# kch3782/torcwa

Measured on AMD Instinct MI355X. Metric: RCWA layer-solves/sec (complex64 I/O) at Fourier order [15,15], higher is better.
Workload: dtype c128 results (mixed-precision eigensolver: fp32 eigendecomposition refined to fp64 by two Newton steps -- fp64 residual and update GEMMs, the correction solved with ONE fp32 LU of the fp32 start; everything else fp64 MFMA); complex64 I/O; 1 GPU; configs[1]: single patterned layer, order=[15,15] (n=1922), 300x300 grid, 128-lambda sweep, glass input half-space; points_total=128, points_per_gpu=128, layer_solves_per_point=1, chunk=128, streams=1, precision=high

## Files before the change

include/trx.h:

```cpp
#ifndef TRX_H_
#define TRX_H_
#include <stddef.h>

#ifdef __cplusplus
extern "C" {
#endif

enum { TRX_C64 = 0, TRX_C128 = 1 };
enum { TRX_OP_N = 0, TRX_OP_T = 1, TRX_OP_C = 2 };
enum {
    TRX_OK = 0,
    TRX_ERR_DTYPE = -1,
    TRX_ERR_ARG = -2,
    TRX_ERR_WORKSPACE = -3,
    TRX_ERR_LAUNCH = -4,
    TRX_ERR_UNSUPPORTED = -5
};

int trx_version(void);
const char* trx_strerror(int code);

size_t trx_convmat_ws_bytes(int dtype, int batch, int nx, int ny, int ox, int oy);
int trx_convmat(int dtype, int grid_is_complex, const void* grid, int batch, int nx, int ny, int ox, int oy,
                void* out, void* ws, size_t ws_bytes, void* stream);
// ... 29 lines not shown
size_t trx_eig_ws_bytes(int dtype, int n, int batch);
int trx_eig(int dtype, void* A, void* w, void* V, int n, int batch, int* info, void* ws, size_t ws_bytes,
            void* stream);
int trx_eig_last_fallback(void);
size_t trx_eig_ws_bytes_opts(int dtype, int n, int batch, unsigned opts);
int trx_eig_opts(int dtype, void* A, void* w, void* V, int n, int batch, int* info, void* ws, size_t ws_bytes, void* stream, unsigned opts);

int trx_tuning(const char* key, int value);

size_t trx_eig_backward_ws_bytes(int dtype, int n, int batch);
int trx_eig_backward(int dtype, const void* w, const void* V, const void* gw, const void* gV, double broadening, int n, int batch,
                     void* gA, int* piv, int* info, void* ws, size_t ws_bytes, void* stream);

int trx_build_pq(int dtype, const void* E, const void* Einv, const void* Mu, const void* Muinv, const void* kx,
                 const void* ky, int N, int batch, void* P, void* Q, void* stream);

size_t trx_layer_smatrix_ws_bytes(int dtype, int N, int batch);
size_t trx_layer_smatrix_ws_bytes_lean(int dtype, int N, int batch);
size_t trx_hmodes_ws_bytes(int dtype, int N, int batch);
int trx_hmodes(int dtype, const void* E, const void* mu, const void* kx, const void* ky, const void* W, const void* kz, int N, int batch,
               void* V, int* piv, int* info, void* ws, size_t ws_bytes, void* stream);
int trx_layer_smatrix(int dtype, const void* P, const void* Q, const void* W, const void* kzfac, const void* vfinv,
                      const void* phase, int use_q, int N, int batch, void* S11, void* S21, void* V, void* Cplus,
                      void* Cminus, int* piv, int* info, void* ws, size_t ws_bytes, void* stream);

size_t trx_redheffer_ws_bytes(int dtype, int n, int batch);
int trx_redheffer(int dtype, const void* const* Sm, const void* const* Sn, void* const* Sout, void* XY, int n, int batch,
                  int* piv, int* info, void* ws, size_t ws_bytes, void* stream);

size_t trx_redheffer_halfspace_ws_bytes(int dtype, int N, int batch, int side, int want_xy);
int trx_redheffer_halfspace(int dtype, int side, const void* bd, const void* const* S, void* const* Sout, void* XY, int N, int batch,
                            int* piv, int* info, void* ws, size_t ws_bytes, void* stream);

size_t trx_build_a_ws_bytes(int dtype, int N, int batch);
int trx_build_a(int dtype, const void* E, const void* Einv, const void* mu, const void* kx, const void* ky, int N, int batch, void* A,
                void* ws, size_t ws_bytes, void* stream);

int trx_build_pq_aniso(int dtype, const void* Ex, const void* Ey, const void* Einv, const void* Mx, const void* My, const void* Minv,
                       const void* kx, const void* ky, int N, int batch, void* P, void* Q, void* stream);
size_t trx_build_a_aniso_ws_bytes(int dtype, int N, int batch);
int trx_build_a_aniso(int dtype, const void* Ex, const void* Ey, const void* Einv, const void* mu, const void* kx, const void* ky, int N, int batch,
                      void* A, void* ws, size_t ws_bytes, void* stream);

int trx_build_pq_tensor(int dtype, const void* Exx, const void* Exy, const void* Eyy, const void* Einv, const void* Mu, const void* Muinv,
                        const void* kx, const void* ky, int N, int batch, void* P, void* Q, void* stream);
size_t trx_build_a_tensor_ws_bytes(int dtype, int N, int batch);
int trx_build_a_tensor(int dtype, const void* Exx, const void* Exy, const void* Eyy, const void* Einv, const void* mu, const void* kx, const void* ky,
                       int N, int batch, void* A, void* ws, size_t ws_bytes, void* stream);

int trx_matvec(int dtype, const void* A, const void* X, long strideX, void* Y, int m, int k, int c, int batch, void* stream);
size_t trx_layer_flux_ws_bytes(int dtype, int N, int nz, int batch);
int trx_layer_flux(int dtype, const void* W, const void* V, const void* cplus, const void* cminus, const void* kz, const double* omega,
                   const double* d, const double* z, int z_is_fraction, int N, int nz, int batch, double* flux, void* ws, size_t ws_bytes,
                   void* stream);

int trx_prof_enable(int on);
int trx_prof_reset(void);
int trx_prof_get(int tag, double* out);
const char* trx_prof_tag_name(int tag);

#ifdef __cplusplus
}
#endif
#endif
```

torcwa_amd/_lib.py:

```python
import ctypes
import os
from ctypes import c_char_p, c_double, c_int, c_long, c_size_t, c_void_p

_HERE = os.path.dirname(os.path.abspath(__file__))
LIB_PATH = os.path.join(_HERE, "libtrx.so")

C64, C128 = 0, 1
OP_N, OP_T, OP_C = 0, 1, 2

_SIGS = {
    "trx_version": (c_int, []),
    "trx_strerror": (c_char_p, [c_int]),
    "trx_convmat_ws_bytes": (c_size_t, [c_int, c_int, c_int, c_int, c_int, c_int]),
    "trx_convmat": (c_int, [c_int, c_int, c_void_p, c_int, c_int, c_int, c_int, c_int, c_void_p, c_void_p, c_size_t, c_void_p]),
    "trx_convmat_orders_ws_bytes": (c_size_t, [c_int, c_int, c_int, c_int, c_int, c_int, c_int]),
    "trx_convmat_orders": (c_int, [c_int, c_int, c_void_p, c_int, c_int, c_int, c_void_p, c_int, c_int, c_int, c_void_p, c_void_p, c_size_t,
                                   c_void_p]),
    "trx_convmat_li_ws_bytes": (c_size_t, [c_int, c_int, c_int, c_int, c_int, c_int]),
    "trx_convmat_li": (c_int, [c_int, c_int, c_void_p, c_int, c_int, c_int, c_int, c_int, c_void_p, c_void_p, c_void_p, c_void_p, c_void_p,
                               c_void_p, c_size_t, c_void_p]),
    "trx_build_pq_aniso": (c_int, [c_int, c_void_p, c_void_p, c_void_p, c_void_p, c_void_p, c_void_p, c_void_p, c_void_p, c_int, c_int, c_void_p,
                                   c_void_p, c_void_p]),
    "trx_build_a_aniso_ws_bytes": (c_size_t, [c_int, c_int, c_int]),
    "trx_build_a_aniso": (c_int, [c_int, c_void_p, c_void_p, c_void_p, c_void_p, c_void_p, c_void_p, c_int, c_int, c_void_p, c_void_p, c_size_t,
# ... 1 lines not shown
    "trx_normal_field_ws_bytes": (c_size_t, [c_int, c_int, c_int, c_int]),
    "trx_normal_field": (c_int, [c_int, c_int, c_void_p, c_int, c_int, c_int, c_double, c_double, c_double, c_void_p, c_void_p, c_size_t, c_void_p]),
    "trx_convmat_nv_ws_bytes": (c_size_t, [c_int, c_int, c_int, c_int, c_int, c_int]),
    "trx_convmat_nv": (c_int, [c_int, c_int, c_void_p, c_int, c_int, c_int, c_int, c_int, c_double, c_double, c_double, c_void_p, c_void_p, c_void_p,
                               c_void_p, c_void_p, c_void_p, c_size_t, c_void_p]),
    "trx_normal_field_lattice": (c_int, [c_int, c_int, c_void_p, c_int, c_int, c_int, c_double, c_void_p, c_void_p, c_void_p, c_size_t, c_void_p]),
    "trx_convmat_nv_orders_ws_bytes": (c_size_t, [c_int, c_int, c_int, c_int, c_int, c_int, c_int]),
    "trx_convmat_nv_orders": (c_int, [c_int, c_int, c_void_p, c_int, c_int, c_int, c_void_p, c_int, c_int, c_int, c_double, c_void_p, c_void_p,
                                      c_void_p, c_void_p, c_void_p, c_void_p, c_void_p, c_size_t, c_void_p]),
    "trx_build_pq_tensor": (c_int, [c_int, c_void_p, c_void_p, c_void_p, c_void_p, c_void_p, c_void_p, c_void_p, c_void_p, c_int, c_int, c_void_p,
                                    c_void_p, c_void_p]),
    "trx_build_a_tensor_ws_bytes": (c_size_t, [c_int, c_int, c_int]),
    "trx_build_a_tensor": (c_int, [c_int, c_void_p, c_void_p, c_void_p, c_void_p, c_void_p, c_void_p, c_void_p, c_int, c_int, c_void_p, c_void_p,
                                   c_size_t, c_void_p]),
    "trx_gemm": (c_int, [c_int, c_int, c_int, c_int, c_int, c_int, c_void_p, c_void_p, c_int, c_long, c_void_p, c_int, c_long,
                         c_void_p, c_void_p, c_int, c_long, c_int, c_void_p]),
    "trx_lu_solve": (c_int, [c_int, c_void_p, c_int, c_void_p, c_int, c_int, c_void_p, c_void_p, c_void_p]),
    "trx_inverse_ws_bytes": (c_size_t, [c_int, c_int, c_int]),
    "trx_inverse": (c_int, [c_int, c_void_p, c_int, c_int, c_void_p, c_void_p, c_void_p, c_size_t, c_void_p]),
    "trx_eig_ws_bytes": (c_size_t, [c_int, c_int, c_int]),
    "trx_build_pq": (c_int, [c_int, c_void_p, c_void_p, c_void_p, c_void_p, c_void_p, c_void_p, c_int, c_int, c_void_p, c_void_p, c_void_p]),
    "trx_layer_smatrix_ws_bytes": (c_size_t, [c_int, c_int, c_int]),
    "trx_layer_smatrix_ws_bytes_lean": (c_size_t, [c_int, c_int, c_int]),
    "trx_layer_smatrix": (c_int, [c_int, c_void_p, c_void_p, c_void_p, c_void_p, c_void_p, c_void_p, c_int, c_int, c_int, c_void_p, c_void_p,
                                  c_void_p, c_void_p, c_void_p, c_void_p, c_void_p, c_void_p, c_size_t, c_void_p]),
    "trx_eig_backward_ws_bytes": (c_size_t, [c_int, c_int, c_int]),
    "trx_eig_backward": (c_int, [c_int, c_void_p, c_void_p, c_void_p, c_void_p, c_double, c_int, c_int, c_void_p, c_void_p, c_void_p, c_void_p, c_size_t, c_void_p]),
    "trx_hmodes_ws_bytes": (c_size_t, [c_int, c_int, c_int]),
    "trx_hmodes": (c_int, [c_int, c_void_p, c_void_p, c_void_p, c_void_p, c_void_p, c_void_p, c_int, c_int, c_void_p, c_void_p, c_void_p, c_void_p, c_size_t, c_void_p]),
    "trx_redheffer_ws_bytes": (c_size_t, [c_int, c_int, c_int]),
    "trx_redheffer": (c_int, [c_int, c_void_p, c_void_p, c_void_p, c_void_p, c_int, c_int, c_void_p, c_void_p, c_void_p, c_size_t, c_void_p]),
    "trx_redheffer_halfspace_ws_bytes": (c_size_t, [c_int, c_int, c_int, c_int, c_int]),
    "trx_redheffer_halfspace": (c_int, [c_int, c_int, c_void_p, c_void_p, c_void_p, c_void_p, c_int, c_int, c_void_p, c_void_p, c_void_p, c_size_t, c_void_p]),
    "trx_build_a_ws_bytes": (c_size_t, [c_int, c_int, c_int]),
    "trx_build_a": (c_int, [c_int, c_void_p, c_void_p, c_void_p, c_void_p, c_void_p, c_int, c_int, c_void_p, c_void_p, c_size_t, c_void_p]),
    "trx_matvec": (c_int, [c_int, c_void_p, c_void_p, c_long, c_void_p, c_int, c_int, c_int, c_int, c_void_p]),
    "trx_layer_flux_ws_bytes": (c_size_t, [c_int, c_int, c_int, c_int]),
    "trx_layer_flux": (c_int, [c_int, c_void_p, c_void_p, c_void_p, c_void_p, c_void_p, c_void_p, c_void_p, c_void_p, c_int, c_int, c_int, c_int,
                               c_void_p, c_void_p, c_size_t, c_void_p]),
    "trx_tuning": (c_int, [c_char_p, c_int]),
    "trx_prof_enable": (c_int, [c_int]),
    "trx_prof_reset": (c_int, []),
    "trx_prof_get": (c_int, [c_int, c_void_p]),
    "trx_prof_tag_name": (c_char_p, [c_int]),
    "trx_eig": (c_int, [c_int, c_void_p, c_void_p, c_void_p, c_int, c_int, c_void_p, c_void_p, c_size_t, c_void_p]),
    "trx_eig_last_fallback": (c_int, []),
    "trx_eig_ws_bytes_opts": (c_size_t, [c_int, c_int, c_int, ctypes.c_uint]),
    "trx_eig_opts": (c_int, [c_int, c_void_p, c_void_p, c_void_p, c_int, c_int, c_void_p, c_void_p, c_size_t, c_void_p, ctypes.c_uint]),
}


class TrxError(RuntimeError):
    pass


class TrxLib:

    def __init__(self, path):
        if not os.path.exists(path):
            raise TrxError(
                f"{path} not found: the HIP extension is not built. Run `python torcwa_amd/csrc/build.py` "
                "(hipcc --offload-arch=gfx950). torcwa_amd has no CPU fallback.")
        self.path = path
        self.dll = ctypes.CDLL(path)
        for name, (res, args) in _SIGS.items():
            fn = getattr(self.dll, name)
# ... 22 lines not shown
```

torcwa_amd/batched.py:

```python
import warnings

import numpy as np
import torch

from .engine import Engine, default_engine
from . import autograd_ops as ag
from . import lattice as _lat
from .flux import FluxMixin
from .torch_eig import Eig

PI_REF = 3.141592652589793

_DIRS = {"f": "forward", "forward": "forward", "b": "backward", "backward": "backward"}
_PORTS = {"t": "transmission", "transmission": "transmission", "r": "reflection", "reflection": "reflection"}
_SBLOCK = {("forward", "transmission"): 0, ("forward", "reflection"): 1, ("backward", "reflection"): 2, ("backward", "transmission"): 3}
_KZ_SIDES = {0: ("out", "in"), 1: ("in", "in"), 2: ("out", "out"), 3: ("in", "out")}
FOURIER_RULES = ("laurent", "li", "normal")
NV_SIGMA_DEFAULT = 6.0


def check_fourier_rule(rule):
    if rule not in FOURIER_RULES:
        raise ValueError(f"fourier_rule must be one of {FOURIER_RULES}, got {rule!r}")

# ... 547 lines not shown
                Cn[1].append(eng.gemm(C[1][m], Y2.contiguous()))
        return Sn, Cn

    @staticmethod
    def _is_bd(S):
        return isinstance(S[0], BlockDiag2)

    @staticmethod
    def _RS_bd_bd(Sm, Sn):
        one, zero = torch.ones_like(Sm[0].d[0]), torch.zeros_like(Sm[0].d[0])
        I = BlockDiag2(one, zero, zero, one)
        t1 = (I - Sm[2] @ Sn[1]).inv()
        t2 = (I - Sn[1] @ Sm[2]).inv()
        return [Sn[0] @ t1 @ Sm[0], Sm[1] + Sm[3] @ t2 @ Sn[1] @ Sm[0], Sn[2] + Sn[0] @ t1 @ Sm[2] @ Sn[3], Sm[3] @ t2 @ Sn[3]]

    def _star(self, Sm, Sn, Cm, Cn):
        bm, bn = self._is_bd(Sm), self._is_bd(Sn)
        if bm and bn:
            return self._RS_bd_bd(Sm, Sn), [[], []]
        if bm:
            return self._RS_halfspace(0, Sm, Sn, Cn)
        if bn:
            return self._RS_halfspace(1, Sn, Sm, Cm)
        return self._RS_prod(Sm, Sn, Cm, Cn)

    def _layer_S(self, i):
        return [self.layer_S11[i], self.layer_S21[i], self.layer_S21[i], self.layer_S11[i]]

    def _layer_C(self, i):
        if not self.keep_coupling or self.Cplus[i] is None:
            return [[], []]
        return [[torch.cat((self.Cplus[i], self.Cminus[i]), dim=1)], [torch.cat((self.Cminus[i], self.Cplus[i]), dim=1)]]

    def solve_global_smatrix(self):
        n, B = self.n, self.B
        self._zero_layer_S = False
        first = 1
        if self._n_folded > 0:
            S, C, first = self._running, [[], []], self._n_folded
        elif self.layer_N > 0:
            S = self._layer_S(0)
            C = self._layer_C(0)
        else:
            I = torch.eye(n, dtype=self._cdtype, device=self._device).expand(B, -1, -1).contiguous()
            Z = torch.zeros((B, n, n), dtype=self._cdtype, device=self._device)
            S = [I, Z, Z.clone(), I.clone()]
            C = [[], []]
            self._zero_layer_S = not (self.has_in or self.has_out)
        for i in range(first, self.layer_N):
            S, C = self._star(S, self._layer_S(i), C, self._layer_C(i))
        if self.has_in:
            S, C = self._star(self._Sin, S, [[], []], C)
        if self.has_out:
            S, C = self._star(S, self._Sout, C, [[], []])
        if self._is_bd(S):
            S = [blk.dense().to(self._cdtype) for blk in S]
        self.S = S
        self.C = C

    def _matching_indices(self, orders):
        if self._general:
            idx = []
            for p, q in orders.reshape(-1, 2).tolist():
                if (p, q) not in self._index:
                    raise ValueError(f"harmonic ({p}, {q}) is not in this solver's order set")
                idx.append(self._index[(p, q)])
            return torch.as_tensor(idx, dtype=torch.int64, device=orders.device)
        ox, oy = self.order
        orders[orders[:, 0] < -ox, 0] = -ox
        orders[orders[:, 0] > ox, 0] = ox
        orders[orders[:, 1] < -oy, 1] = -oy
        orders[orders[:, 1] > oy, 1] = oy
        return len(self.order_y) * (orders[:, 0] + ox) + orders[:, 1] + oy

    def _kz_real(self, side, evan, abs_when_evanescent=False):
        em = self.eps_in * self.mu_in if side == "in" else self.eps_out * self.mu_out
        kzc = torch.sqrt(em[:, None] - self.Kx_norm_dn ** 2 - self.Ky_norm_dn ** 2)
        ev = torch.abs(torch.real(kzc) / torch.imag(kzc)) < evan
        repl = torch.abs(torch.real(kzc)) if abs_when_evanescent else torch.zeros_like(torch.real(kzc))
        kz = torch.where(ev, repl, torch.real(kzc))
        return torch.cat((kz, kz), dim=1)

    def S_parameters(self, orders, *, direction="forward", port="transmission", polarization="xx", ref_order=[0, 0],
                     power_norm=True, evanscent=1e-3):
        dev = self._device
        orders = torch.as_tensor(orders, dtype=torch.int64, device=dev).reshape([-1, 2])
        if direction in _DIRS:
            direction = _DIRS[direction]
        else:
            warnings.warn("Invalid propagation direction. Set as forward.", UserWarning)
            direction = "forward"
        if port in _PORTS:
            port = _PORTS[port]
        else:
            warnings.warn("Invalid port. Set as tramsmission.", UserWarning)
            port = "transmission"
        if polarization not in ("xx", "yx", "xy", "yy", "pp", "sp", "ps", "ss"):
            warnings.warn("Invalid polarization. Set as xx.", UserWarning)
            polarization = "xx"
        ref_order = torch.as_tensor(ref_order, dtype=torch.int64, device=dev).reshape([1, 2])
        oi = self._matching_indices(orders)
        ri = self._matching_indices(ref_order)
        N = self.order_N
        k = _SBLOCK[(direction, port)]
        Sk = self.S[k]
        num_side, den_side = _KZ_SIDES[k]

        if polarization in ("xx", "yx", "xy", "yy"):
            if polarization[0] == "y":
                oi = oi + N
            if polarization[1] == "y":
                ri = ri + N
            val = Sk[:, oi, ri[0]]
            if power_norm:
                kzn, kzd = self._kz_real(num_side, evanscent), self._kz_real(den_side, evanscent)
                kxr = torch.cat((torch.real(self.Kx_norm_dn),) * 2, dim=1)
                kyr = torch.cat((torch.real(self.Ky_norm_dn),) * 2, dim=1)
                pn = kxr if polarization[0] == "x" else kyr
                pd = kxr if polarization[1] == "x" else kyr
                norm = torch.sqrt((1 + (pn[:, oi] / kzn[:, oi]) ** 2) / (1 + (pd[:, ri] / kzd[:, ri]) ** 2))
                norm = norm * torch.sqrt(kzn[:, oi] / kzd[:, ri])
                val = val * norm
            val = torch.where(torch.isinf(val), torch.zeros_like(val), val)
            val = torch.where(torch.isnan(val), torch.zeros_like(val), val)
            return val.to(self._dtype)

        osign, rsign = {0: (1, 1), 1: (-1, 1), 2: (1, -1), 3: (-1, -1)}[k]
        em_in, em_out = self.eps_in * self.mu_in, self.eps_out * self.mu_out
        ok2 = {0: em_out, 1: em_in, 2: em_out, 3: em_in}[k]
        rk2 = {0: em_in, 1: em_in, 2: em_out, 3: em_out}[k]

        def angles(idx, k2, sign):
            kx_, ky_ = self.Kx_norm_dn[:, idx], self.Ky_norm_dn[:, idx]
            kt = torch.sqrt(kx_ ** 2 + ky_ ** 2)
            kzc = torch.sqrt(k2[:, None] - kx_ ** 2 - ky_ ** 2)
            kzs = sign * torch.abs(torch.real(kzc))
            ev = torch.abs(torch.real(kzc) / torch.imag(kzc)) < evanscent
            return torch.atan2(torch.real(kt), kzs), torch.atan2(torch.real(ky_), torch.real(kx_)), ev

        o_inc, o_azi, o_ev = angles(oi, ok2, osign)
        r_inc, r_azi, r_ev = angles(ri, rk2, rsign)
        r0 = int(ri[0])
        xx, xy = Sk[:, oi, r0], Sk[:, oi, r0 + N]
        yx, yy = Sk[:, oi + N, r0], Sk[:, oi + N, r0 + N]
        zero = torch.zeros_like(xx)
        xx, xy, yx, yy = (torch.where(o_ev, zero, t) for t in (xx, xy, yx, yy))
        co, so, ci = torch.cos(o_azi), torch.sin(o_azi), torch.cos(o_inc)
        cr, sr, cri = torch.cos(r_azi), torch.sin(r_azi), torch.cos(r_inc)
        if polarization == "pp":
            val = co / ci * cri * cr * xx + so / ci * cri * cr * yx + co / ci * cri * sr * xy + so / ci * cri * sr * yy
        elif polarization == "ps":
            val = co / ci * (-1) * sr * xx + so / ci * (-1) * sr * yx + co / ci * cr * xy + so / ci * cr * yy
        elif polarization == "sp":
            val = -so * cri * cr * xx + co * cri * cr * yx + -so * cri * sr * xy + co * cri * sr * yy
        else:
            val = -so * (-1) * sr * xx + co * (-1) * sr * yx + -so * cr * xy + co * cr * yy
        val = torch.where(torch.isinf(val), torch.zeros_like(val), val)
        val = torch.where(torch.isnan(val), torch.zeros_like(val), val)
        if power_norm:
            kz_in = self._kz_real("in", evanscent)
            kz_out = self._kz_real("out", evanscent, abs_when_evanescent=True)
            kzn = kz_out if num_side == "out" else kz_in
            kzd = kz_out if den_side == "out" else kz_in
            val = val * torch.sqrt(kzn[:, oi] / kzd[:, ri])
        val = torch.where(r_ev, torch.zeros_like(val), val)
        return val.to(self._dtype)

    def diffraction_angle(self, orders, *, layer="output", unit="radian"):
        orders = torch.as_tensor(orders, dtype=torch.int64, device=self._device).reshape([-1, 2])
        if layer in ("i", "in", "input"):
            layer = "input"
        elif layer in ("o", "out", "output"):
            layer = "output"
        else:
            warnings.warn("Invalid layer. Set as output layer.", UserWarning)
            layer = "output"
        if unit in ("r", "rad", "radian"):
# ... 18 lines not shown
```

torcwa_amd/csrc/api.hip:

```cpp
#include "common.hpp"

using namespace trx;

extern "C" int trx_version(void) { return 500; }

extern "C" const char* trx_strerror(int code) {
    switch (code) {
        case TRX_OK: return "ok";
        case TRX_ERR_DTYPE: return "unsupported dtype (expected TRX_C64 or TRX_C128)";
        case TRX_ERR_ARG: return "invalid argument";
        case TRX_ERR_WORKSPACE: return "workspace too small";
        case TRX_ERR_LAUNCH: return "kernel launch failed";
        case TRX_ERR_UNSUPPORTED: return "unsupported problem size or option";
        default: return code > 0 ? "numerical failure (see info[])" : "unknown error";
    }
}

namespace {
template <class T>
__global__ __launch_bounds__(256) void set_identity_kernel(cx<T>* __restrict__ X, int n) {
    cx<T>* M = X + (long)blockIdx.z * n * n;
    const int j = blockIdx.x * blockDim.x + threadIdx.x;
    const int i = blockIdx.y;
    if (j < n) M[(long)i * n + j] = cx<T>(i == j ? T(1) : T(0), T(0));
}

template <class T>
int inverse_t(hipStream_t s, cx<T>* A, int n, int batch, int* piv, int* info, cx<T>* ws) {
    const long nn = (long)n * n;
    int rc = lu_factor<T>(s, A, n, nn, n, piv, batch, info);
    if (rc) return rc;
    TRX_LAUNCH((set_identity_kernel<T>), dim3(cdiv_i(n, 256), n, batch), dim3(256), 0, s, ws, n);
    rc = lu_solve<T>(s, A, n, nn, n, piv, ws, n, nn, n, batch);
    if (rc) return rc;
    if (hipMemcpyAsync(A, ws, sizeof(cx<T>) * nn * batch, hipMemcpyDeviceToDevice, s) != hipSuccess) return TRX_ERR_LAUNCH;
    return TRX_OK;
}
// ... 46 lines not shown
```

torcwa_amd/csrc/smatrix.hip:

```cpp
#include "common.hpp"

namespace trx {
namespace {

template <class T>
__global__ __launch_bounds__(256) void build_pq_kernel(const cx<T>* __restrict__ E, const cx<T>* __restrict__ Ei,
                                                       const cx<T>* __restrict__ M, const cx<T>* __restrict__ Mi,
                                                       const cx<T>* __restrict__ kx, const cx<T>* __restrict__ ky, int N,
                                                       cx<T>* __restrict__ P, cx<T>* __restrict__ Q) {
    const int b = blockIdx.z, i = blockIdx.y;
    const int j = blockIdx.x * blockDim.x + threadIdx.x;
    if (j >= N) return;
    const long o = ((long)b * N + i) * N + j;
    const cx<T> e = E[o], ei = Ei[o], m = M[o], mi = Mi[o];
    const cx<T> kxi = kx[(long)b * N + i], kyi = ky[(long)b * N + i], kxj = kx[(long)b * N + j], kyj = ky[(long)b * N + j];
    const int n = 2 * N;
    cx<T>* Pb = P + (long)b * n * n;
    cx<T>* Qb = Q + (long)b * n * n;
    const long r0 = (long)i * n + j, r1 = (long)(i + N) * n + j;
    Pb[r0] = kxi * ei * kyj;
    Pb[r0 + N] = m - kxi * ei * kxj;
    Pb[r1] = kyi * ei * kyj - m;
    Pb[r1 + N] = -(kyi * ei * kxj);
    Qb[r0] = -(kxi * mi * kyj);
// ... 346 lines not shown
        TRX_LAUNCH((bd_dense_kernel<T>), gn, blk, 0, s, D11, bN, (const cx<T>*)nullptr, 0, 0L, X, 2 * n, 2 * nn, N);
        TRX_LAUNCH((bd_rowcomb_kernel<T>), gN, blk, 0, s, D12, bN, S[3], n, nn, (const cx<T>*)nullptr, 0, 0L, X + n, 2 * n, 2 * nn, N, n, T(1), 0);
        rc = lu_factor<T>(s, K, n, nn, n, piv, batch, info); if (rc) return rc;
        rc = lu_solve<T>(s, K, n, nn, n, piv, X, 2 * n, 2 * nn, 2 * n, batch); if (rc) return rc;
        rc = gemm<T>(s, TRX_OP_N, TRX_OP_N, n, n, n, one, S[0], n, nn, X, 2 * n, 2 * nn, zero, O[0], n, nn, batch); if (rc) return rc;
        TRX_LAUNCH((block_copy_kernel<T>), gn, blk, 0, s, S[2], n, nn, O[2], n, nn, n, n, T(1), 0);
        rc = gemm<T>(s, TRX_OP_N, TRX_OP_N, n, n, n, one, S[0], n, nn, X + n, 2 * n, 2 * nn, one, O[2], n, nn, batch); if (rc) return rc;
        rc = gemm<T>(s, TRX_OP_N, TRX_OP_N, n, n, n, one, S[1], n, nn, X, 2 * n, 2 * nn, zero, Y, 2 * n, 2 * nn, batch); if (rc) return rc;
        TRX_LAUNCH((block_copy_kernel<T>), gn, blk, 0, s, S[3], n, nn, Y + n, 2 * n, 2 * nn, n, n, T(1), 0);
        rc = gemm<T>(s, TRX_OP_N, TRX_OP_N, n, n, n, one, S[1], n, nn, X + n, 2 * n, 2 * nn, one, Y + n, 2 * n, 2 * nn, batch); if (rc) return rc;
        TRX_LAUNCH((bd_dense_kernel<T>), gn, blk, 0, s, D21, bN, (const cx<T>*)nullptr, 0, 0L, O[1], n, nn, N);
        TRX_LAUNCH((bd_rowcomb_kernel<T>), gN, blk, 0, s, D22, bN, (const cx<T>*)Y, 2 * n, 2 * nn, (const cx<T>*)O[1], n, nn, O[1], n, nn, N, n, T(1), 0);
        TRX_LAUNCH((bd_rowcomb_kernel<T>), gN, blk, 0, s, D22, bN, (const cx<T>*)(Y + n), 2 * n, 2 * nn, (const cx<T>*)nullptr, 0, 0L, O[3], n, nn, N, n, T(1), 0);
    } else {
        TRX_LAUNCH((bd_colcomb_kernel<T>), gc, blk, 0, s, D21, bN, S[2], n, nn, K, n, nn, N, n, T(-1), 1);
        TRX_LAUNCH((block_copy_kernel<T>), gn, blk, 0, s, S[0], n, nn, X, 2 * n, 2 * nn, n, n, T(1), 0);
        TRX_LAUNCH((bd_colcomb_kernel<T>), gc, blk, 0, s, D22, bN, S[2], n, nn, X + n, 2 * n, 2 * nn, N, n, T(1), 0);
        rc = lu_factor<T>(s, K, n, nn, n, piv, batch, info); if (rc) return rc;
        rc = lu_solve<T>(s, K, n, nn, n, piv, X, 2 * n, 2 * nn, 2 * n, batch); if (rc) return rc;
        TRX_LAUNCH((bd_rowcomb_kernel<T>), gN, blk, 0, s, D11, bN, (const cx<T>*)X, 2 * n, 2 * nn, (const cx<T>*)nullptr, 0, 0L, O[0], n, nn, N, n, T(1), 0);
        TRX_LAUNCH((bd_dense_kernel<T>), gn, blk, 0, s, D12, bN, (const cx<T>*)nullptr, 0, 0L, O[2], n, nn, N);
        TRX_LAUNCH((bd_rowcomb_kernel<T>), gN, blk, 0, s, D11, bN, (const cx<T>*)(X + n), 2 * n, 2 * nn, (const cx<T>*)O[2], n, nn, O[2], n, nn, N, n, T(1), 0);
        TRX_LAUNCH((bd_rowcomb_kernel<T>), gN, blk, 0, s, D21, bN, (const cx<T>*)X, 2 * n, 2 * nn, (const cx<T>*)nullptr, 0, 0L, Y, 2 * n, 2 * nn, N, n, T(1), 0);
        TRX_LAUNCH((bd_dense_kernel<T>), gn, blk, 0, s, D22, bN, (const cx<T>*)nullptr, 0, 0L, Y + n, 2 * n, 2 * nn, N);
        TRX_LAUNCH((bd_rowcomb_kernel<T>), gN, blk, 0, s, D21, bN, (const cx<T>*)(X + n), 2 * n, 2 * nn, (const cx<T>*)(Y + n), 2 * n, 2 * nn, Y + n, 2 * n, 2 * nn, N, n, T(1), 0);
        TRX_LAUNCH((block_copy_kernel<T>), gn, blk, 0, s, S[1], n, nn, O[1], n, nn, n, n, T(1), 0);
        rc = gemm<T>(s, TRX_OP_N, TRX_OP_N, n, n, n, one, S[3], n, nn, Y, 2 * n, 2 * nn, one, O[1], n, nn, batch); if (rc) return rc;
        rc = gemm<T>(s, TRX_OP_N, TRX_OP_N, n, n, n, one, S[3], n, nn, Y + n, 2 * n, 2 * nn, zero, O[3], n, nn, batch); if (rc) return rc;
    }
    TRX_CHECK_LAUNCH();
    return TRX_OK;
}

template <class T>
__global__ __launch_bounds__(256) void scale_rows_kernel(const cx<T>* __restrict__ in, const cx<T>* __restrict__ s, int N, cx<T>* __restrict__ out) {
    const int b = blockIdx.z, i = blockIdx.y;
    const int j = blockIdx.x * blockDim.x + threadIdx.x;
    if (j >= N) return;
    const long o = ((long)b * N + i) * N + j;
    out[o] = s[(long)b * N + i] * in[o];
}
template <class T>
__global__ __launch_bounds__(256) void assemble_a_kernel(const cx<T>* __restrict__ E, const cx<T>* __restrict__ Gx, const cx<T>* __restrict__ Gy,
                                                         const cx<T>* __restrict__ mu, const cx<T>* __restrict__ kx, const cx<T>* __restrict__ ky, int N,
                                                         cx<T>* __restrict__ A) {
    const int b = blockIdx.z, i = blockIdx.y;
    const int j = blockIdx.x * blockDim.x + threadIdx.x;
    if (j >= N) return;
    const long o = ((long)b * N + i) * N + j;
    const cx<T> kxi = kx[(long)b * N + i], kyi = ky[(long)b * N + i];
    const cx<T> e = mu[b] * E[o], gx = Gx[o], gy = Gy[o];
    const int n = 2 * N;
    cx<T>* Ab = A + (long)b * n * n;
    cx<T> a11 = e - kxi * gx, a12 = -(kxi * gy), a21 = -(kyi * gx), a22 = e - kyi * gy;
    if (i == j) { a11 -= kyi * kyi; a22 -= kxi * kxi; a12 += kxi * kyi; a21 += kxi * kyi; }
    Ab[(long)i * n + j] = a11;
    Ab[(long)i * n + j + N] = a12;
    Ab[(long)(i + N) * n + j] = a21;
    Ab[(long)(i + N) * n + j + N] = a22;
}
template <class T>
int build_a_t(hipStream_t s, const cx<T>* E, const cx<T>* Ei, const cx<T>* mu, const cx<T>* kx, const cx<T>* ky, int N, int batch, cx<T>* A, cx<T>* ws) {
    const long NN = (long)N * N, bNN = (long)batch * NN;
    const cx<T> one(T(1), T(0)), zero(T(0), T(0));
    const dim3 g(cdiv_i(N, 256), N, batch), blk(256);
    cx<T>*Sx = ws, *Gx = ws + bNN, *Gy = ws + 2 * bNN;
// ... 72 lines not shown
    return (size_t)(dtype == TRX_C128 ? 16 : 8) * (size_t)batch * (size_t)n * n;
}

extern "C" int trx_redheffer(int dtype, const void* const* Sm, const void* const* Sn, void* const* Sout, void* XY, int n, int batch,
                             int* piv, int* info, void* ws, size_t ws_bytes, void* stream) {
    if (!Sm || !Sn || !Sout || !XY || !piv || !info || !ws || n <= 0 || batch <= 0) return TRX_ERR_ARG;
    for (int k = 0; k < 4; ++k)
        if (!Sm[k] || !Sn[k] || !Sout[k]) return TRX_ERR_ARG;
    if (ws_bytes < trx_redheffer_ws_bytes(dtype, n, batch)) return TRX_ERR_WORKSPACE;
    hipStream_t s = trx::api_stream(stream);
    if (dtype == TRX_C64) return redheffer_t<float>(s, (const cx<float>* const*)Sm, (const cx<float>* const*)Sn, (cx<float>* const*)Sout, (cx<float>*)XY, n, batch, piv, info, (cx<float>*)ws);
    if (dtype == TRX_C128) return redheffer_t<double>(s, (const cx<double>* const*)Sm, (const cx<double>* const*)Sn, (cx<double>* const*)Sout, (cx<double>*)XY, n, batch, piv, info, (cx<double>*)ws);
    return TRX_ERR_DTYPE;
}

extern "C" size_t trx_redheffer_halfspace_ws_bytes(int dtype, int N, int batch, int side, int want_xy) {
    const size_t nn = (size_t)(dtype == TRX_C128 ? 16 : 8) * (size_t)batch * (size_t)(2 * N) * (size_t)(2 * N);
    return (side == 0 && !want_xy) ? 4 * nn : nn;
}

extern "C" int trx_redheffer_halfspace(int dtype, int side, const void* bd, const void* const* S, void* const* Sout, void* XY, int N, int batch,
                                       int* piv, int* info, void* ws, size_t ws_bytes, void* stream) {
    if (!bd || !S || !Sout || !piv || !info || !ws || N <= 0 || batch <= 0 || (side != 0 && side != 1)) return TRX_ERR_ARG;
    if (!XY && side == 1) return TRX_ERR_ARG;
    for (int k = 0; k < 4; ++k)
        if (!S[k] || !Sout[k]) return TRX_ERR_ARG;
    if (ws_bytes < trx_redheffer_halfspace_ws_bytes(dtype, N, batch, side, XY != nullptr)) return TRX_ERR_WORKSPACE;
    hipStream_t s = trx::api_stream(stream);
    if (dtype == TRX_C64) return redheffer_halfspace_t<float>(s, side, (const cx<float>*)bd, (const cx<float>* const*)S, (cx<float>* const*)Sout, (cx<float>*)XY, N, batch, piv, info, (cx<float>*)ws);
    if (dtype == TRX_C128) return redheffer_halfspace_t<double>(s, side, (const cx<double>*)bd, (const cx<double>* const*)S, (cx<double>* const*)Sout, (cx<double>*)XY, N, batch, piv, info, (cx<double>*)ws);
    return TRX_ERR_DTYPE;
}

extern "C" size_t trx_build_a_ws_bytes(int dtype, int N, int batch) {
    return (size_t)(dtype == TRX_C128 ? 16 : 8) * 3 * (size_t)batch * N * N;
}

extern "C" int trx_build_a(int dtype, const void* E, const void* Einv, const void* mu, const void* kx, const void* ky, int N, int batch, void* A,
                           void* ws, size_t ws_bytes, void* stream) {
    if (!E || !Einv || !mu || !kx || !ky || !A || !ws || N <= 0 || batch <= 0) return TRX_ERR_ARG;
    if (ws_bytes < trx_build_a_ws_bytes(dtype, N, batch)) return TRX_ERR_WORKSPACE;
    hipStream_t s = trx::api_stream(stream);
    if (dtype == TRX_C64) return build_a_t<float>(s, (const cx<float>*)E, (const cx<float>*)Einv, (const cx<float>*)mu, (const cx<float>*)kx, (const cx<float>*)ky, N, batch, (cx<float>*)A, (cx<float>*)ws);
    if (dtype == TRX_C128) return build_a_t<double>(s, (const cx<double>*)E, (const cx<double>*)Einv, (const cx<double>*)mu, (const cx<double>*)kx, (const cx<double>*)ky, N, batch, (cx<double>*)A, (cx<double>*)ws);
    return TRX_ERR_DTYPE;
}
```

torcwa_amd/engine.py:

```python
import ctypes
import os
import threading

import torch

from . import _lib

_CODE = {torch.complex64: _lib.C64, torch.complex128: _lib.C128}
_REAL = {torch.complex64: torch.float32, torch.complex128: torch.float64}


class NumericalError(RuntimeError):
    pass


def _phase(name):
    def deco(fn):
        def wrapped(self, *a, **kw):
            if not self.profile_phases or self.device.type != "cuda":
                return fn(self, *a, **kw)
            e0, e1 = torch.cuda.Event(enable_timing=True), torch.cuda.Event(enable_timing=True)
            e0.record(torch.cuda.current_stream(self.device))
            try:
                return fn(self, *a, **kw)
# ... 352 lines not shown
        ws = self._ws(nws)
        arr = ctypes.c_void_p * 4
        pm, pn, po = arr(*[t.data_ptr() for t in Sm]), arr(*[t.data_ptr() for t in Sn]), arr(*[t.data_ptr() for t in out])
        self.lib.check(self.lib.redheffer(_CODE[dt], ctypes.addressof(pm), ctypes.addressof(pn), ctypes.addressof(po), XY.data_ptr(), n, B,
                                          piv.data_ptr(), info.data_ptr(), ws.data_ptr(), nws, self.stream))
        self._info(info, "redheffer")
        X, Y = XY[0], XY[1]
        return out, X[:, :, :n], X[:, :, n:], Y[:, :, :n], Y[:, :, n:]


    @_phase("Redheffer star products")
    def redheffer_halfspace(self, side, bd, S, want_xy=True):
        S = [self._c(t) for t in S]
        B, n, _ = S[0].shape
        N = n // 2
        dt = S[0].dtype
        bd = self._c(bd.to(dt))
        out = [torch.empty((B, n, n), dtype=dt, device=self.device) for _ in range(4)]
        lean = (int(side) == 0) and not want_xy
        XY = None if lean else torch.empty((2, B, n, 2 * n), dtype=dt, device=self.device)
        piv, info = self._ints(B * n), self._ints(B)
        nws = self.lib.redheffer_halfspace_ws_bytes(_CODE[dt], N, B, int(side), 0 if lean else 1)
        ws = self._ws(nws)
        arr = ctypes.c_void_p * 4
        ps, po = arr(*[t.data_ptr() for t in S]), arr(*[t.data_ptr() for t in out])
        self.lib.check(self.lib.redheffer_halfspace(_CODE[dt], int(side), bd.data_ptr(), ctypes.addressof(ps), ctypes.addressof(po),
                                                    None if lean else XY.data_ptr(), N, B, piv.data_ptr(), info.data_ptr(), ws.data_ptr(), nws, self.stream))
        self._info(info, "redheffer_halfspace")
        if lean:
            return out, None, None, None, None
        X, Y = XY[0], XY[1]
        return out, X[:, :, :n], X[:, :, n:], Y[:, :, :n], Y[:, :, n:]

    @_phase("assembly (convolution matrices, E^-1, A = PQ)")
    def build_a(self, E, Einv, mu, kx, ky):
        B, N, _ = E.shape
        dt = E.dtype
        A = torch.empty((B, 2 * N, 2 * N), dtype=dt, device=self.device)
        nws = self.lib.build_a_ws_bytes(_CODE[dt], N, B)
        ws = self._ws(nws)
        self.lib.check(self.lib.build_a(_CODE[dt], self._c(E).data_ptr(), self._c(Einv).data_ptr(), self._c(mu.to(dt)).data_ptr(), self._c(kx).data_ptr(),
                                        self._c(ky).data_ptr(), N, B, A.data_ptr(), ws.data_ptr(), nws, self.stream))
        return A

    @_phase("assembly (convolution matrices, E^-1, A = PQ)")
    def build_pq_aniso(self, Ex, Ey, Einv, Mx, My, Minv, kx, ky):
        B, N, _ = Ex.shape
        dt = Ex.dtype
        P = torch.empty((B, 2 * N, 2 * N), dtype=dt, device=self.device)
        Q = torch.empty_like(P)
        ops = [self._c(t) for t in (Ex, Ey, Einv, Mx, My, Minv, kx, ky)]
        self._check(*ops)
        self.lib.check(self.lib.build_pq_aniso(_CODE[dt], *[t.data_ptr() for t in ops], N, B, P.data_ptr(), Q.data_ptr(), self.stream))
        return P, Q

    @_phase("assembly (convolution matrices, E^-1, A = PQ)")
    def build_a_aniso(self, Ex, Ey, Einv, mu, kx, ky):
        B, N, _ = Ex.shape
        dt = Ex.dtype
        A = torch.empty((B, 2 * N, 2 * N), dtype=dt, device=self.device)
        nws = self.lib.build_a_aniso_ws_bytes(_CODE[dt], N, B)
        ws = self._ws(nws)
        ops = [self._c(t) for t in (Ex, Ey, Einv, mu.to(dt), kx, ky)]
        self._check(*ops)
        self.lib.check(self.lib.build_a_aniso(_CODE[dt], *[t.data_ptr() for t in ops], N, B, A.data_ptr(), ws.data_ptr(), nws, self.stream))
        return A
# ... 66 lines not shown
```

torcwa_amd/sweep.py:

```python
import os

import numpy as np
import torch

from .batched import NV_SIGMA_DEFAULT, BatchedRCWA, check_fourier_rule
from .lattice import parse_order

_DATA = os.path.join(os.path.dirname(os.path.abspath(__file__)), "data")


def shard_range(n_items, rank, world):
    base, rem = divmod(int(n_items), int(world))
    lo = rank * base + min(rank, rem)
    return lo, lo + base + (1 if rank < rem else 0)


def shard_indices(n_items, rank, world, cyclic=False):
    if cyclic:
        return np.arange(int(rank), int(n_items), int(world), dtype=np.int64)
    lo, hi = shard_range(n_items, rank, world)
    return np.arange(lo, hi, dtype=np.int64)


def gather_sweep(local, n_items, group=None, cyclic=False):
# ... 17 lines not shown
        t = out[r][: hi - lo]
        parts.append(torch.view_as_complex(t) if pad.is_complex() else t)
    full = torch.cat(parts, dim=0)
    if not cyclic:
        return full
    order = np.concatenate([shard_indices(n_items, r, world, True) for r in range(world)])
    inv = torch.as_tensor(np.argsort(order), device=full.device)
    return full.index_select(0, inv)


def asih_eps_table():
    z = np.load(os.path.join(_DATA, "asih_eps_400_700_128.npz"))
    return z["lam"], z["eps"]


def rectangle_density(nx, ny, Lx, Ly, Wx, Wy, Cx, Cy, theta=0.0, edge_sharpness=1000.0, dtype=torch.float64, device="cpu"):
    from .geometry import geometry
    g = geometry(Lx=Lx, Ly=Ly, nx=nx, ny=ny, edge_sharpness=edge_sharpness, dtype=dtype, device=torch.device(device))
    return g.rectangle(Wx=Wx, Wy=Wy, Cx=Cx, Cy=Cy, theta=theta)


def _solve_chunk(freq, layers, order, L, eps_in, eps_out, inc_ang, azi_ang, dtype, precision, engine, orders,
                 polarization, direction, port, check_info, eig_route="auto", route_hint=None, fourier_rule="laurent", nv_sigma=NV_SIGMA_DEFAULT,
                 absorption=False, source=None):
    sim = BatchedRCWA(freq, order, L, dtype=dtype, precision=precision, engine=engine, keep_coupling=bool(absorption), fold_layers=not absorption,
                      eig_route=eig_route, route_hint=route_hint, fourier_rule=fourier_rule, nv_sigma=nv_sigma)
    if eps_in is not None:
        sim.add_input_layer(eps=eps_in)
    if eps_out is not None:
        sim.add_output_layer(eps=eps_out)
    sim.set_incident_angle(inc_ang, azi_ang)
    for lay in layers:
        sim.add_layer(*lay)
    sim.solve_global_smatrix()
    sp = sim.S_parameters([list(o) for o in orders], direction=direction, port=port, polarization=polarization)
    if not absorption:
        return sp
    src = dict(amplitude=[1.0, 0.0], notation="xy", direction=direction)
    src.update(source or {})
    if "orders" in src:
        sim.source_fourier(**src)
    else:
        sim.source_planewave(**src)
    return sp, sim.absorption()


_POINT_MATRICES = {1: 15.0, 2: 18.0}
_LI_EXTRA = 0.5
_NV_EXTRA = 2.0
_HEADROOM = 0.10


_ABS_EXTRA_PER_LAYER = 15.0


def auto_chunk(B, order, n_layers, precision, device, dtype=torch.complex64, streams=1, fourier_rule="laurent", absorption=False):
    if device.type != "cuda":
        return B
    kind, box, mn = parse_order(order)
    n = 2 * (2 * box[0] + 1) * (2 * box[1] + 1) if kind == "rect" else 2 * len(mn)
    elem = 8 if (precision == "native" and dtype == torch.complex64) else 16
    mats = _POINT_MATRICES[1 if n_layers <= 1 else 2] + {"li": _LI_EXTRA, "normal": _NV_EXTRA}.get(fourier_rule, 0.0)
    if absorption:
        mats += _ABS_EXTRA_PER_LAYER * max(1, int(n_layers))
    per_point = mats * n * n * elem * max(1, int(streams))
    free, total = torch.cuda.mem_get_info(device)
    free += torch.cuda.memory_reserved(device) - torch.cuda.memory_allocated(device)
    budget = free - _HEADROOM * total
    fit = int(budget // per_point)
    if fit < 1:
# ... 99 lines not shown
```

Measured before the change: 38.32 layer-solves/s.

## Compute only needed S-matrix columns in the final half-space Redheffer product

When only S-parameters are requested, the sweep now defers the last half-space star product and calls a new kernel path. That path factors the coupling matrix once, then solves and multiplies only for the few reference columns needed, instead of forming the full dense output blocks. This replaces full-matrix LU solves and GEMMs on 2N-wide right-hand sides with matvec-sized work on at most 16 columns. The full global S-matrix is no longer stored on this path, and a new API plus extra kernels must be kept consistent with the dense version.

```diff
diff --git a/include/trx.h b/include/trx.h
--- a/include/trx.h
+++ b/include/trx.h
@@ -85,6 +85,10 @@
 int trx_redheffer_halfspace(int dtype, int side, const void* bd, const void* const* S, void* const* Sout, void* XY, int N, int batch,
                             int* piv, int* info, void* ws, size_t ws_bytes, void* stream);
 
+size_t trx_redheffer_halfspace_columns_ws_bytes(int dtype, int N, int batch, int m);
+int trx_redheffer_halfspace_columns(int dtype, int side, const void* bd, const void* const* S, int block, const int* cols, int m, void* out,
+                                    int N, int batch, int* piv, int* info, void* ws, size_t ws_bytes, void* stream);
+
 size_t trx_build_a_ws_bytes(int dtype, int N, int batch);
 int trx_build_a(int dtype, const void* E, const void* Einv, const void* mu, const void* kx, const void* ky, int N, int batch, void* A,
                 void* ws, size_t ws_bytes, void* stream);
diff --git a/torcwa_amd/_lib.py b/torcwa_amd/_lib.py
--- a/torcwa_amd/_lib.py
+++ b/torcwa_amd/_lib.py
@@ -57,6 +57,9 @@
     "trx_redheffer": (c_int, [c_int, c_void_p, c_void_p, c_void_p, c_void_p, c_int, c_int, c_void_p, c_void_p, c_void_p, c_size_t, c_void_p]),
     "trx_redheffer_halfspace_ws_bytes": (c_size_t, [c_int, c_int, c_int, c_int, c_int]),
     "trx_redheffer_halfspace": (c_int, [c_int, c_int, c_void_p, c_void_p, c_void_p, c_void_p, c_int, c_int, c_void_p, c_void_p, c_void_p, c_size_t, c_void_p]),
+    "trx_redheffer_halfspace_columns_ws_bytes": (c_size_t, [c_int, c_int, c_int, c_int]),
+    "trx_redheffer_halfspace_columns": (c_int, [c_int, c_int, c_void_p, c_void_p, c_int, c_void_p, c_int, c_void_p, c_int, c_int, c_void_p, c_void_p,
+                                                c_void_p, c_size_t, c_void_p]),
     "trx_build_a_ws_bytes": (c_size_t, [c_int, c_int, c_int]),
     "trx_build_a": (c_int, [c_int, c_void_p, c_void_p, c_void_p, c_void_p, c_void_p, c_int, c_int, c_void_p, c_void_p, c_size_t, c_void_p]),
     "trx_matvec": (c_int, [c_int, c_void_p, c_void_p, c_long, c_void_p, c_int, c_int, c_int, c_int, c_void_p]),
diff --git a/torcwa_amd/batched.py b/torcwa_amd/batched.py
--- a/torcwa_amd/batched.py
+++ b/torcwa_amd/batched.py
@@ -603,7 +603,7 @@
             return [[], []]
         return [[torch.cat((self.Cplus[i], self.Cminus[i]), dim=1)], [torch.cat((self.Cminus[i], self.Cplus[i]), dim=1)]]
 
-    def solve_global_smatrix(self):
+    def _cascade(self, defer_last=False):
         n, B = self.n, self.B
         self._zero_layer_S = False
         first = 1
@@ -620,14 +620,36 @@
             self._zero_layer_S = not (self.has_in or self.has_out)
         for i in range(first, self.layer_N):
             S, C = self._star(S, self._layer_S(i), C, self._layer_C(i))
-        if self.has_in:
-            S, C = self._star(self._Sin, S, [[], []], C)
-        if self.has_out:
-            S, C = self._star(S, self._Sout, C, [[], []])
+        sides = ([0] if self.has_in else []) + ([1] if self.has_out else [])
+        for j, side in enumerate(sides):
+            if (defer_last and j == len(sides) - 1 and not self.keep_coupling and not getattr(self, "_diff", False)
+                    and not self._is_bd(S) and not C[0] and not C[1]):
+                return S, C, side
+            S, C = self._star(self._Sin, S, [[], []], C) if side == 0 else self._star(S, self._Sout, C, [[], []])
+        return S, C, None
+
+    def solve_global_smatrix(self):
+        S, C, _ = self._cascade()
         if self._is_bd(S):
             S = [blk.dense().to(self._cdtype) for blk in S]
         self.S = S
         self.C = C
+
+    def solve_S_parameters(self, orders, *, direction="forward", port="transmission", polarization="xx", ref_order=[0, 0],
+                           power_norm=True, evanscent=1e-3):
+        orders, polarization, oi, ri, k = self._sparam_args(orders, direction, port, polarization, ref_order)
+        S, C, side = self._cascade(defer_last=True)
+        if side is None:
+            if self._is_bd(S):
+                S = [blk.dense().to(self._cdtype) for blk in S]
+            self.S, self.C = S, C
+            Sk = S[k]
+            return self._sparam_values(lambda c: Sk[:, :, c], k, oi, ri, polarization, power_norm, evanscent)
+        cols = self._sparam_columns(ri, polarization)
+        Sbd = self._Sin if side == 0 else self._Sout
+        bd = torch.stack([torch.stack(blk.d, dim=0) for blk in Sbd], dim=0).to(self._cdtype).contiguous()
+        out = self.engine.redheffer_halfspace_columns(side, bd, S, k, cols)
+        return self._sparam_values(lambda c: out[:, :, cols.index(c)], k, oi, ri, polarization, power_norm, evanscent)
 
     def _matching_indices(self, orders):
         if self._general:
@@ -652,8 +674,7 @@
         kz = torch.where(ev, repl, torch.real(kzc))
         return torch.cat((kz, kz), dim=1)
 
-    def S_parameters(self, orders, *, direction="forward", port="transmission", polarization="xx", ref_order=[0, 0],
-                     power_norm=True, evanscent=1e-3):
+    def _sparam_args(self, orders, direction, port, polarization, ref_order):
         dev = self._device
         orders = torch.as_tensor(orders, dtype=torch.int64, device=dev).reshape([-1, 2])
         if direction in _DIRS:
@@ -672,9 +693,22 @@
         ref_order = torch.as_tensor(ref_order, dtype=torch.int64, device=dev).reshape([1, 2])
         oi = self._matching_indices(orders)
         ri = self._matching_indices(ref_order)
+        return orders, polarization, oi, ri, _SBLOCK[(direction, port)]
+
+    def _sparam_columns(self, ri, polarization):
+        r0 = int(ri[0])
+        if polarization in ("xx", "yx", "xy", "yy"):
+            return [r0 + (self.order_N if polarization[1] == "y" else 0)]
+        return [r0, r0 + self.order_N]
+
+    def S_parameters(self, orders, *, direction="forward", port="transmission", polarization="xx", ref_order=[0, 0],
+                     power_norm=True, evanscent=1e-3):
+        orders, polarization, oi, ri, k = self._sparam_args(orders, direction, port, polarization, ref_order)
+        Sk = self.S[k]
+        return self._sparam_values(lambda c: Sk[:, :, c], k, oi, ri, polarization, power_norm, evanscent)
+
+    def _sparam_values(self, col, k, oi, ri, polarization, power_norm, evanscent):
         N = self.order_N
-        k = _SBLOCK[(direction, port)]
-        Sk = self.S[k]
         num_side, den_side = _KZ_SIDES[k]
 
         if polarization in ("xx", "yx", "xy", "yy"):
@@ -682,7 +716,7 @@
                 oi = oi + N
             if polarization[1] == "y":
                 ri = ri + N
-            val = Sk[:, oi, ri[0]]
+            val = col(int(ri[0]))[:, oi]
             if power_norm:
                 kzn, kzd = self._kz_real(num_side, evanscent), self._kz_real(den_side, evanscent)
                 kxr = torch.cat((torch.real(self.Kx_norm_dn),) * 2, dim=1)
@@ -712,8 +746,9 @@
         o_inc, o_azi, o_ev = angles(oi, ok2, osign)
         r_inc, r_azi, r_ev = angles(ri, rk2, rsign)
         r0 = int(ri[0])
-        xx, xy = Sk[:, oi, r0], Sk[:, oi, r0 + N]
-        yx, yy = Sk[:, oi + N, r0], Sk[:, oi + N, r0 + N]
+        c0, c1 = col(r0), col(r0 + N)
+        xx, xy = c0[:, oi], c1[:, oi]
+        yx, yy = c0[:, oi + N], c1[:, oi + N]
         zero = torch.zeros_like(xx)
         xx, xy, yx, yy = (torch.where(o_ev, zero, t) for t in (xx, xy, yx, yy))
         co, so, ci = torch.cos(o_azi), torch.sin(o_azi), torch.cos(o_inc)
diff --git a/torcwa_amd/csrc/api.hip b/torcwa_amd/csrc/api.hip
--- a/torcwa_amd/csrc/api.hip
+++ b/torcwa_amd/csrc/api.hip
@@ -2,7 +2,7 @@
 
 using namespace trx;
 
-extern "C" int trx_version(void) { return 500; }
+extern "C" int trx_version(void) { return 600; }
 
 extern "C" const char* trx_strerror(int code) {
     switch (code) {
diff --git a/torcwa_amd/csrc/smatrix.hip b/torcwa_amd/csrc/smatrix.hip
--- a/torcwa_amd/csrc/smatrix.hip
+++ b/torcwa_amd/csrc/smatrix.hip
@@ -402,6 +402,120 @@
     return TRX_OK;
 }
 
+constexpr int PROBE_MAX_COLS = 16;
+struct ProbeCols { int c[PROBE_MAX_COLS]; };
+
+template <class T>
+__device__ inline cx<T> bd_elem(const cx<T>* __restrict__ d, long dstride, int b, int N, int i, int j) {
+    const int ii = i < N ? i : i - N, jj = j < N ? j : j - N;
+    if (ii != jj) return cx<T>(T(0), T(0));
+    return d[(long)((i < N ? 0 : 2) + (j < N ? 0 : 1)) * dstride + (long)b * N + ii];
+}
+template <class T>
+__device__ inline cx<T> probe_col_elem(const cx<T>* __restrict__ A, const cx<T>* __restrict__ Dr, long dstride, int b, int N, int r, int c) {
+    const int n = 2 * N;
+    if (!A) return bd_elem(Dr, dstride, b, N, r, c);
+    const cx<T>* Ar = A + ((long)b * n + r) * n;
+    if (!Dr) return Ar[c];
+    const int jj = c < N ? c : c - N;
+    return Ar[jj] * bd_elem(Dr, dstride, b, N, jj, c) + Ar[jj + N] * bd_elem(Dr, dstride, b, N, jj + N, c);
+}
+template <class T>
+__global__ __launch_bounds__(256) void probe_col_kernel(const cx<T>* __restrict__ Dl, const cx<T>* __restrict__ A, const cx<T>* __restrict__ Dr,
+                                                        long dstride, ProbeCols cols, int m, int N, cx<T>* __restrict__ out) {
+    const int b = blockIdx.z, q = blockIdx.y, n = 2 * N;
+    const int i = blockIdx.x * blockDim.x + threadIdx.x;
+    if (i >= n) return;
+    const int c = cols.c[q];
+    cx<T> v;
+    if (!Dl) {
+        v = probe_col_elem(A, Dr, dstride, b, N, i, c);
+    } else {
+        const int ii = i < N ? i : i - N;
+        v = bd_elem(Dl, dstride, b, N, i, ii) * probe_col_elem(A, Dr, dstride, b, N, ii, c)
+          + bd_elem(Dl, dstride, b, N, i, ii + N) * probe_col_elem(A, Dr, dstride, b, N, ii + N, c);
+    }
+    out[((long)b * n + i) * m + q] = v;
+}
+template <class T>
+__global__ __launch_bounds__(256) void probe_comb_kernel(const cx<T>* __restrict__ D, long dstride, const cx<T>* X, const cx<T>* Y, int m, int N,
+                                                         cx<T>* out) {
+    const int b = blockIdx.z, i = blockIdx.y, n = 2 * N;
+    const int q = blockIdx.x * blockDim.x + threadIdx.x;
+    if (q >= m) return;
+    const long o = ((long)b * n + i) * m + q;
+    cx<T> v;
+    if (D) {
+        const int ii = i < N ? i : i - N;
+        v = bd_elem(D, dstride, b, N, i, ii) * X[((long)b * n + ii) * m + q] + bd_elem(D, dstride, b, N, i, ii + N) * X[((long)b * n + ii + N) * m + q];
+    } else {
+        v = X[o];
+    }
+    if (Y) v += Y[o];
+    out[o] = v;
+}
+
+template <class T>
+int redheffer_halfspace_columns_t(hipStream_t s, int dtype, int side, const cx<T>* bd, const cx<T>* const* S, int block, const int* cols, int m,
+                                  cx<T>* out, int N, int batch, int* piv, int* info, cx<T>* ws) {
+    const int n = 2 * N;
+    const long nn = (long)n * n, bn = (long)batch * nn, bN = (long)batch * N, bv = (long)batch * n * m;
+    const dim3 blk(256), gN(cdiv_i(n, 256), N, batch), gc(cdiv_i(N, 256), n, batch), gp(cdiv_i(n, 256), m, batch), gv(cdiv_i(m, 256), n, batch);
+    const cx<T>*D11 = bd, *D21 = bd + 4 * bN, *D12 = bd + 8 * bN, *D22 = bd + 12 * bN;
+    const cx<T>* const nul = nullptr;
+    cx<T>* K = ws;
+    cx<T>* U = ws + bn;
+    cx<T>* Tv = U + bv;
+    cx<T>* Yv = Tv + bv;
+    ProbeCols pc;
+    for (int q = 0; q < PROBE_MAX_COLS; ++q) pc.c[q] = q < m ? cols[q] : 0;
+    const bool right = block >= 2;
+    int rc;
+    auto matvec = [&](const cx<T>* A, const cx<T>* X, cx<T>* Y) { return trx_matvec(dtype, A, X, (long)n * m, Y, n, n, m, batch, (void*)s); };
+    if (side == 0) {
+        TRX_LAUNCH((bd_rowcomb_kernel<T>), gN, blk, 0, s, D12, bN, S[1], n, nn, nul, 0, 0L, K, n, nn, N, n, T(-1), 1);
+        if (!right) TRX_LAUNCH((probe_col_kernel<T>), gp, blk, 0, s, nul, nul, D11, bN, pc, m, N, U);
+        else        TRX_LAUNCH((probe_col_kernel<T>), gp, blk, 0, s, D12, S[3], nul, bN, pc, m, N, U);
+        rc = lu_factor<T>(s, K, n, nn, n, piv, batch, info); if (rc) return rc;
+        rc = lu_solve<T>(s, K, n, nn, n, piv, U, m, (long)n * m, m, batch); if (rc) return rc;
+        if (block == 0) return matvec(S[0], U, out);
+        rc = matvec(S[(block == 2) ? 0 : 1], U, Tv); if (rc) return rc;
+        if (block == 1) {
+            TRX_LAUNCH((probe_col_kernel<T>), gp, blk, 0, s, nul, nul, D21, bN, pc, m, N, Yv);
+            TRX_LAUNCH((probe_comb_kernel<T>), gv, blk, 0, s, D22, bN, (const cx<T>*)Tv, (const cx<T>*)Yv, m, N, out);
+        } else if (block == 2) {
+            TRX_LAUNCH((probe_col_kernel<T>), gp, blk, 0, s, nul, S[2], nul, bN, pc, m, N, Yv);
+            TRX_LAUNCH((probe_comb_kernel<T>), gv, blk, 0, s, nul, bN, (const cx<T>*)Tv, (const cx<T>*)Yv, m, N, out);
+        } else {
+            TRX_LAUNCH((probe_col_kernel<T>), gp, blk, 0, s, D22, S[3], nul, bN, pc, m, N, Yv);
+            TRX_LAUNCH((probe_comb_kernel<T>), gv, blk, 0, s, D22, bN, (const cx<T>*)Tv, (const cx<T>*)Yv, m, N, out);
+        }
+    } else {
+        TRX_LAUNCH((bd_colcomb_kernel<T>), gc, blk, 0, s, D21, bN, S[2], n, nn, K, n, nn, N, n, T(-1), 1);
+        if (!right) TRX_LAUNCH((probe_col_kernel<T>), gp, blk, 0, s, nul, S[0], nul, bN, pc, m, N, U);
+        else        TRX_LAUNCH((probe_col_kernel<T>), gp, blk, 0, s, nul, S[2], D22, bN, pc, m, N, U);
+        rc = lu_factor<T>(s, K, n, nn, n, piv, batch, info); if (rc) return rc;
+        rc = lu_solve<T>(s, K, n, nn, n, piv, U, m, (long)n * m, m, batch); if (rc) return rc;
+        if (block == 0) {
+            TRX_LAUNCH((probe_comb_kernel<T>), gv, blk, 0, s, D11, bN, (const cx<T>*)U, nul, m, N, out);
+        } else if (block == 2) {
+            TRX_LAUNCH((probe_col_kernel<T>), gp, blk, 0, s, nul, nul, D12, bN, pc, m, N, Yv);
+            TRX_LAUNCH((probe_comb_kernel<T>), gv, blk, 0, s, D11, bN, (const cx<T>*)U, (const cx<T>*)Yv, m, N, out);
+        } else if (block == 1) {
+            TRX_LAUNCH((probe_comb_kernel<T>), gv, blk, 0, s, D21, bN, (const cx<T>*)U, nul, m, N, Tv);
+            rc = matvec(S[3], Tv, U); if (rc) return rc;
+            TRX_LAUNCH((probe_col_kernel<T>), gp, blk, 0, s, nul, S[1], nul, bN, pc, m, N, Yv);
+            TRX_LAUNCH((probe_comb_kernel<T>), gv, blk, 0, s, nul, bN, (const cx<T>*)U, (const cx<T>*)Yv, m, N, out);
+        } else {
+            TRX_LAUNCH((probe_col_kernel<T>), gp, blk, 0, s, nul, nul, D22, bN, pc, m, N, Yv);
+            TRX_LAUNCH((probe_comb_kernel<T>), gv, blk, 0, s, D21, bN, (const cx<T>*)U, (const cx<T>*)Yv, m, N, Tv);
+            return matvec(S[3], Tv, out);
+        }
+    }
+    TRX_CHECK_LAUNCH();
+    return TRX_OK;
+}
+
 template <class T>
 __global__ __launch_bounds__(256) void scale_rows_kernel(const cx<T>* __restrict__ in, const cx<T>* __restrict__ s, int N, cx<T>* __restrict__ out) {
     const int b = blockIdx.z, i = blockIdx.y;
@@ -540,6 +654,29 @@
     return TRX_ERR_DTYPE;
 }
 
+extern "C" size_t trx_redheffer_halfspace_columns_ws_bytes(int dtype, int N, int batch, int m) {
+    const size_t n = 2 * (size_t)N;
+    return (size_t)(dtype == TRX_C128 ? 16 : 8) * (size_t)batch * (n * n + 3 * n * (size_t)m);
+}
+
+extern "C" int trx_redheffer_halfspace_columns(int dtype, int side, const void* bd, const void* const* S, int block, const int* cols, int m,
+                                               void* out, int N, int batch, int* piv, int* info, void* ws, size_t ws_bytes, void* stream) {
+    if (!bd || !S || !cols || !out || !piv || !info || !ws || N <= 0 || batch <= 0 || batch > 65535 || (side != 0 && side != 1)) return TRX_ERR_ARG;
+    if (block < 0 || block > 3 || m < 1 || m > PROBE_MAX_COLS) return TRX_ERR_ARG;
+    for (int k = 0; k < 4; ++k)
+        if (!S[k]) return TRX_ERR_ARG;
+    for (int q = 0; q < m; ++q)
+        if (cols[q] < 0 || cols[q] >= 2 * N) return TRX_ERR_ARG;
+    if (dtype != TRX_C64 && dtype != TRX_C128) return TRX_ERR_DTYPE;
+    if (ws_bytes < trx_redheffer_halfspace_columns_ws_bytes(dtype, N, batch, m)) return TRX_ERR_WORKSPACE;
+    hipStream_t s = trx::api_stream(stream);
+    if (dtype == TRX_C64)
+        return redheffer_halfspace_columns_t<float>(s, dtype, side, (const cx<float>*)bd, (const cx<float>* const*)S, block, cols, m, (cx<float>*)out, N, batch,
+                                                    piv, info, (cx<float>*)ws);
+    return redheffer_halfspace_columns_t<double>(s, dtype, side, (const cx<double>*)bd, (const cx<double>* const*)S, block, cols, m, (cx<double>*)out, N, batch,
+                                                 piv, info, (cx<double>*)ws);
+}
+
 extern "C" size_t trx_build_a_ws_bytes(int dtype, int N, int batch) {
     return (size_t)(dtype == TRX_C128 ? 16 : 8) * 3 * (size_t)batch * N * N;
 }
diff --git a/torcwa_amd/engine.py b/torcwa_amd/engine.py
--- a/torcwa_amd/engine.py
+++ b/torcwa_amd/engine.py
@@ -408,6 +408,27 @@
         X, Y = XY[0], XY[1]
         return out, X[:, :, :n], X[:, :, n:], Y[:, :, :n], Y[:, :, n:]
 
+    @_phase("Redheffer star products")
+    def redheffer_halfspace_columns(self, side, bd, S, block, cols):
+        S = [self._c(t) for t in S]
+        self._check(*S)
+        B, n, _ = S[0].shape
+        N = n // 2
+        dt = S[0].dtype
+        bd = self._c(bd.to(dt))
+        cols = [int(c) for c in cols]
+        m = len(cols)
+        out = torch.empty((B, n, m), dtype=dt, device=self.device)
+        piv, info = self._ints(B * n), self._ints(B)
+        nws = self.lib.redheffer_halfspace_columns_ws_bytes(_CODE[dt], N, B, m)
+        ws = self._ws(nws)
+        ps = (ctypes.c_void_p * 4)(*[t.data_ptr() for t in S])
+        pc = (ctypes.c_int * max(m, 1))(*cols)
+        self.lib.check(self.lib.redheffer_halfspace_columns(_CODE[dt], int(side), bd.data_ptr(), ctypes.addressof(ps), int(block), ctypes.addressof(pc), m,
+                                                            out.data_ptr(), N, B, piv.data_ptr(), info.data_ptr(), ws.data_ptr(), nws, self.stream))
+        self._info(info, "redheffer_halfspace_columns")
+        return out
+
     @_phase("assembly (convolution matrices, E^-1, A = PQ)")
     def build_a(self, E, Einv, mu, kx, ky):
         B, N, _ = E.shape
diff --git a/torcwa_amd/sweep.py b/torcwa_amd/sweep.py
--- a/torcwa_amd/sweep.py
+++ b/torcwa_amd/sweep.py
@@ -73,10 +73,10 @@
     sim.set_incident_angle(inc_ang, azi_ang)
     for lay in layers:
         sim.add_layer(*lay)
+    if not absorption:
+        return sim.solve_S_parameters([list(o) for o in orders], direction=direction, port=port, polarization=polarization)
     sim.solve_global_smatrix()
     sp = sim.S_parameters([list(o) for o in orders], direction=direction, port=port, polarization=polarization)
-    if not absorption:
-        return sp
     src = dict(amplitude=[1.0, 0.0], notation="xy", direction=direction)
     src.update(source or {})
     if "orders" in src:
```

Result: faster. 43.99 layer-solves/s (median of 6 runs) (+14.8%).
